# OnurBasci/TransformerBasedNavierStokeSolver

Measured on AMD Instinct MI355X. Metric: ns64_train_samples_per_s, higher is better.
Workload: dtype f32

## Files before the change

transformerbasednavierstokesolver_amd/csrc/pa2d_gemm.hip:

```cpp
#include "pa2d_gemm_common.h"
#include <string.h>


static Pa2dEnv read_env() {
    auto is = [](const char* n, const char* pre) { const char* e = getenv(n); return e && strncmp(e, pre, strlen(pre)) == 0; };
    auto num = [](const char* n, int dflt) { const char* e = getenv(n); return (e && e[0]) ? atoi(e) : dflt; };
    Pa2dEnv v;
    v.conv_halo = is("PA2D_CONV_HALO", "o") ? 0 : (is("PA2D_CONV_HALO", "f") ? 2 : 1);
    v.mc_big_off = is("PA2D_MC_BIG", "o") ? 1 : 0;
    v.kc_bk16 = num("PA2D_KC_BK", 0) == 16 ? 1 : 0;
    v.mc_bk = num("PA2D_MC_BK", 16) == 32 ? 32 : 16;
    v.mc_splits = num("PA2D_MC_SPLITS", 0);
    v.mcb_splits = num("PA2D_MCB_SPLITS", 0);
    v.lin_dw_split = is("PA2D_LIN_DW_SPLIT", "of") ? 0 : 1;
    v.lin_panel = is("PA2D_LIN_PANEL", "of") ? 0 : 1;
    v.lin_rowpanel = is("PA2D_LIN_ROWPANEL", "of") ? 0 : 1;
    v.lin_small_split = is("PA2D_LIN_SMALL_SPLIT", "of") ? 0 : 1;
    v.conv_mfma16 = num("PA2D_CONV_MFMA", 16) == 32 ? 0 : 1;
    v.split_big = num("PA2D_SPLIT_BIG", 1);
    v.slice_map = is("PA2D_SLICE_MAP", "l") ? 0 : 1;
    v.default_engine = is("PA2D_GEMM", "f") ? 0 : (is("PA2D_GEMM", "b") ? 2 : 1);
    return v;
}
static Pa2dEnv g_env = read_env();
const Pa2dEnv& pa2d_env() { return g_env; }
static int kc_bk(bool im2col, int Cin) {
    if (im2col && pa2d_env().kc_bk16) return 16;
    return (!im2col || (Cin % 32) == 0) ? 32 : 16;
}
KCTile kc_tile(int M, int N, bool im2col, int Cin) {
    const int tiles_m = ceil_div(M, 128);
    const long long t128 = (long long)tiles_m * ceil_div(N, 128);
    const long long t12864 = (long long)tiles_m * ceil_div(N, 64);
    const int bk = kc_bk(im2col, Cin);
    if (N > 64 && t128 >= 384) return {128, 128, bk};
    if (t12864 >= 384 || M <= 64) return {128, 64, bk};
    return {64, 64, bk};
}
bool use_split(int engine, int N, bool im2col, int Cin) {
    const int m = engine;
    if (m == 1) return im2col && N > 64 && (Cin % 32) == 0;
    if (m == 2) return N > 64 && (!im2col || (Cin % 32) == 0);
    return false;
}

int launch_kc(const KCParams& p_in, bool im2col, hipStream_t st, hipEvent_t ev0, hipEvent_t ev1) {
    KCParams p = p_in;
    if (!engine_ok(p.engine)) return PA2D_ERR_ARG;
    if (p.M <= 0 || p.N <= 0 || p.K <= 0) return PA2D_OK;
    if (!p.bias2) p.bias_split = 0x7fffffff;
    {
        const unsigned long long ab = ((unsigned long long)(p.M - 1) * p.lda + (im2col ? p.Cin : p.K)) * 4ull;
        const unsigned long long bb = ((unsigned long long)(p.N - 1) * p.ldb + p.K) * 4ull;
        if (ab >= 0xFFFFFFF0ull || bb >= 0xFFFFFFF0ull) return PA2D_ERR_UNSUPPORTED;
        p.a_bytes = (unsigned)ab;
        p.b_bytes = (unsigned)bb;
        const unsigned long long es = p.io_bf16 ? 2ull : 4ull;
        const unsigned long long cb = ((unsigned long long)(p.M - 1) * p.ldc + p.N) * es;
        const unsigned long long rb = p.res ? ((unsigned long long)(p.M - 1) * p.ldres + p.N) * es : 0ull;
        const unsigned long long xb = p.aux ? ((unsigned long long)(p.M - 1) * p.ldaux + p.N) * es : 0ull;
        if (cb >= 0xFFFFFFF0ull || rb >= 0xFFFFFFF0ull || xb >= 0xFFFFFFF0ull) return PA2D_ERR_UNSUPPORTED;
        p.c_bytes = (unsigned)cb; p.res_bytes = (unsigned)rb; p.aux_bytes = (unsigned)xb;
    }
    if ((p.K & 3) || (p.lda & 3) || (p.ldb & 3)) return PA2D_ERR_ARG;
    if (im2col && ((p.Cin & 15) || p.K != (p.taps == 27 ? 27 : 9) * p.Cin)) return PA2D_ERR_UNSUPPORTED;
    if (im2col && (p.epi != 0 || p.res)) return PA2D_ERR_ARG;
    if (ev0 && hipEventRecord(ev0, st) != hipSuccess) return PA2D_ERR_ARG;
    int rc;
    if (!im2col && p.wimg && rowpanel_applies(p)) {
        if (p.wsrc) {
            rc = launch_pack_weight_image(p.wsrc, p.wsn, p.wsk, p.wimg, p.N, p.K, st);
            if (rc) return rc;
        }
        KCParams pp = p;
        pp.M = p.M - p.M % 128;
        rc = launch_kc_rowpanel(pp, p.wimg, st);
        if (!rc && pp.M < p.M) {
            KCParams pt = p_in;
            pt.wimg = nullptr;
            pt.M = p.M - pp.M;
            pt.A = p.A + (size_t)pp.M * p.lda;
            pt.C = p.C + (size_t)pp.M * p.ldc;
            if (p.res) pt.res = p.res + (size_t)pp.M * p.ldres;
            if (p.aux) pt.aux = p.aux + (size_t)pp.M * p.ldaux;
            rc = launch_kc(pt, false, st);
        }
    } else if (panel_applies(p, im2col)) {
        KCParams pp = p;
        pp.M = p.M - p.M % 256;
        rc = launch_kc_panel(pp, st);
        if (!rc && pp.M < p.M) {
            KCParams pt = p_in;
            const size_t ea = p.io_bf16 ? 2 : 4, es = p.io_bf16 ? 2 : 4;
            pt.M = p.M - pp.M;
            pt.A = (const float*)((const char*)p.A + (size_t)pp.M * p.lda * ea);
            pt.C = (float*)((char*)p.C + (size_t)pp.M * p.ldc * es);
            if (p.res) pt.res = (const float*)((const char*)p.res + (size_t)pp.M * p.ldres * es);
            if (p.aux) pt.aux = (float*)((char*)p.aux + (size_t)pp.M * p.ldaux * es);
            rc = launch_kc(pt, false, st);
        }
    } else if (p.io_bf16 || use_split(p.engine, p.N, im2col, p.Cin)) rc = launch_kc_split(p, im2col, st);
    else if (kc_split_small_applies(p, im2col)) rc = launch_kc_split_small(p, st);
    else rc = launch_kc_f32(p, im2col, kc_tile(p.M, p.N, im2col, p.Cin), st);
    if (rc) return rc;
    if (ev1 && hipEventRecord(ev1, st) != hipSuccess) return PA2D_ERR_ARG;
    return PA2D_OK;
}

template <int TAPS>
__global__ void repack_kernel(const float* __restrict__ w0, const float* __restrict__ w1, float* __restrict__ dst,
                              int mode, int N, int K, int C, int Cin, int NK) {
    const long long idx = (long long)blockIdx.x * blockDim.x + threadIdx.x;
    if (mode == 0) {
        if (idx >= (long long)N * K) return;
        const int n = (int)(idx % N), k = (int)(idx / N);
        dst[idx] = w0[(size_t)n * K + k];
    } else if (mode == 1) {
        if (idx >= (long long)NK * C * TAPS * Cin) return;
        const int CH = K;
        const int c16 = (int)(idx % CH);
        const int tap = (int)((idx / CH) % TAPS);
        const int cic = (int)((idx / (TAPS * CH)) % (Cin / CH));
        const int co = (int)(idx / ((long long)Cin * TAPS));
        const int ci = cic * CH + c16;
        const float* src = co < C ? w0 : w1;
        dst[idx] = src[((size_t)(co % C) * Cin + ci) * TAPS + tap];
    } else {
        if (idx >= (long long)NK * C * TAPS * Cin) return;
        const int CH = K;
        const int c16 = (int)(idx % CH);
        const int tap = (int)((idx / CH) % TAPS);
        const int cic = (int)((idx / (TAPS * CH)) % (NK * C / CH));
        const int ci = (int)(idx / ((long long)NK * C * TAPS));
        const int co = cic * CH + c16;
        const float* src = co < C ? w0 : w1;
        dst[idx] = src[((size_t)(co % C) * Cin + ci) * TAPS + (TAPS - 1 - tap)];
    }
}

int launch_repack(const float* w0, const float* w1, float* dst, int mode, int N, int K, int C, int Cin, hipStream_t st,
                  int taps) {
    const int nk = w1 ? 2 : 1;
    const long long count = mode == 0 ? (long long)N * K : (long long)nk * C * taps * Cin;
    const dim3 grid((unsigned)ceil_div_ll(count, 256));
    if (taps == 27)
        hipLaunchKernelGGL(repack_kernel<27>, grid, dim3(256), 0, st, w0, w1, dst, mode, N, K, C, Cin, nk);
    else
        hipLaunchKernelGGL(repack_kernel<9>, grid, dim3(256), 0, st, w0, w1, dst, mode, N, K, C, Cin, nk);
    PA2D_CHECK_LAUNCH();
    return PA2D_OK;
}

static KCParams dense_fwd_params(const void* x, long long ldx, const float* w, long long ldw, const float* bias,
                                 const void* res, long long ldres, void* y, long long ldy, void* pre, long long ldpre, int M,
                                 int N, int K, int act, int engine, bool io_bf16) {
    KCParams p = {};
    p.engine = engine; p.io_bf16 = io_bf16 ? 1 : 0; p.apre = io_bf16 ? 1 : 0;
    p.aux_deriv = (act & PA2D_ACT_SAVE_DERIVATIVE_BIT) ? 1 : 0;
    act &= ~PA2D_ACT_SAVE_DERIVATIVE_BIT;
    p.A = (const float*)x; p.lda = ldx; p.B = w; p.ldb = ldw; p.C = (float*)y; p.ldc = ldy; p.bias = bias;
    p.res = (const float*)res; p.ldres = ldres; p.aux = (float*)pre; p.ldaux = ldpre; p.M = M; p.N = N; p.K = K; p.act = act;
    p.epi = (act != ACT_NONE ? EPI_ACT : 0) | (pre ? EPI_STORE_PRE : 0);
    return p;
}
static KCParams dense_bwd_data_params(const void* dy, long long lddy, const float* wt, const void* pre, long long ldpre,
                                      int act, void* dx, long long lddx, int M, int N, int K, int engine, bool io_bf16) {
    KCParams p = {};
    p.engine = engine; p.io_bf16 = io_bf16 ? 1 : 0; p.apre = io_bf16 ? 1 : 0;
    p.aux_deriv = (act & PA2D_ACT_SAVE_DERIVATIVE_BIT) ? 1 : 0;
    act &= ~PA2D_ACT_SAVE_DERIVATIVE_BIT;
    p.A = (const float*)dy; p.lda = lddy; p.B = wt; p.ldb = N; p.C = (float*)dx; p.ldc = lddx; p.M = M; p.N = K; p.K = N;
    p.aux = (float*)const_cast<void*>(pre); p.ldaux = ldpre; p.act = act;
    p.epi = (pre && act != ACT_NONE) ? EPI_MUL_DACT : 0;
// ... 126 lines not shown
```

transformerbasednavierstokesolver_amd/csrc/pa2d_internal.h:

```cpp
#pragma once
#include <hip/hip_runtime.h>
#include <stdint.h>

typedef float f32x16 __attribute__((ext_vector_type(16)));
typedef float f32x4 __attribute__((ext_vector_type(4)));

#define PA2D_OK 0
#define PA2D_ERR_ARG 1001
#define PA2D_ERR_UNSUPPORTED 1002
#define PA2D_ERR_WORKSPACE 1003

#define PA2D_CHECK_LAUNCH()                         \
    do {                                            \
        hipError_t e__ = hipGetLastError();         \
        if (e__ != hipSuccess) return (int)e__;     \
    } while (0)

enum { ACT_NONE = 0, ACT_GELU = 1, ACT_TANH = 2, ACT_SIGMOID = 3, ACT_RELU = 4, ACT_SOFTPLUS = 5,
       ACT_ELU = 6, ACT_SILU = 7 };

__device__ __forceinline__ float normal_cdf(float x, float& e_out) {
#pragma clang fp contract(off)
    const float z = fabsf(x) * 0.70710678118654752440f;
    const float t = __builtin_amdgcn_rcpf(fmaf(0.3275911f, z, 1.0f));
    float poly = fmaf(1.061405429f, t, -1.453152027f);
    poly = fmaf(poly, t, 1.421413741f);
    poly = fmaf(poly, t, -0.284496736f);
    poly = fmaf(poly, t, 0.254829592f);
    const float e = __builtin_amdgcn_exp2f(-z * z * 1.44269504088896340736f);
    e_out = e;
    const float hq = 0.5f * poly * t * e;
    return x < 0.f ? hq : 1.0f - hq;
}
__device__ __forceinline__ float gelu_exact(float x) {
#pragma clang fp contract(off)
    float e;
    return x * normal_cdf(x, e);
}
__device__ __forceinline__ float dgelu_exact(float x) {
#pragma clang fp contract(off)
    float e;
    const float cdf = normal_cdf(x, e);
    return fmaf(x * 0.39894228040143267794f, e, cdf);
}

__device__ __forceinline__ float act_fwd(int id, float x) {
    switch (id) {
        case ACT_GELU: return gelu_exact(x);
        case ACT_TANH: return tanhf(x);
        case ACT_SIGMOID: return 1.0f / (1.0f + expf(-x));
        case ACT_RELU: return x > 0.f ? x : 0.f;
        case ACT_SOFTPLUS: return x > 20.f ? x : log1pf(expf(x));
        case ACT_ELU: return x > 0.f ? x : expm1f(x);
        case ACT_SILU: return x / (1.0f + expf(-x));
        default: return x;
    }
}

__device__ __forceinline__ float act_bwd(int id, float x) {
    switch (id) {
        case ACT_GELU: return dgelu_exact(x);
        case ACT_TANH: { const float t = tanhf(x); return 1.0f - t * t; }
        case ACT_SIGMOID: { const float s = 1.0f / (1.0f + expf(-x)); return s * (1.0f - s); }
        case ACT_RELU: return x > 0.f ? 1.f : 0.f;
        case ACT_SOFTPLUS: return x > 20.f ? 1.f : 1.0f / (1.0f + expf(-x));
        case ACT_ELU: return x > 0.f ? 1.f : expf(x);
        case ACT_SILU: { const float s = 1.0f / (1.0f + expf(-x)); return s * (1.0f + x * (1.0f - s)); }
        default: return 1.f;
    }
}

__device__ __forceinline__ float wave_sum(float v) {
#pragma unroll
    for (int o = 32; o > 0; o >>= 1) v += __shfl_xor(v, o, 64);
    return v;
}
__device__ __forceinline__ float wave_max(float v) {
#pragma unroll
    for (int o = 32; o > 0; o >>= 1) v = fmaxf(v, __shfl_xor(v, o, 64));
    return v;
}

typedef unsigned int u32x4 __attribute__((ext_vector_type(4)));
#define OOB_OFF 0xFFFFFFFFu

__device__ __forceinline__ __amdgpu_buffer_rsrc_t make_rsrc(const float* base, unsigned bytes) {
    return __builtin_amdgcn_make_buffer_rsrc(const_cast<float*>(base), 0, bytes, 0x00020000);
}
__device__ __forceinline__ float4 buf_load4(__amdgpu_buffer_rsrc_t r, unsigned voff) {
    const u32x4 v = __builtin_amdgcn_raw_buffer_load_b128(r, voff, 0, 0);
    return make_float4(__uint_as_float(v.x), __uint_as_float(v.y), __uint_as_float(v.z), __uint_as_float(v.w));
}


__device__ __forceinline__ float buf_load1(__amdgpu_buffer_rsrc_t r, unsigned voff) {
    return __uint_as_float(__builtin_amdgcn_raw_buffer_load_b32(r, voff, 0, 0));
}
__device__ __forceinline__ void buf_store1(__amdgpu_buffer_rsrc_t r, unsigned voff, float v) {
    __builtin_amdgcn_raw_buffer_store_b32(__float_as_uint(v), r, voff, 0, 0);
}

__device__ __forceinline__ float2 buf_load2(__amdgpu_buffer_rsrc_t r, unsigned voff) {
    typedef unsigned int u32x2_ __attribute__((ext_vector_type(2)));
    const u32x2_ v = __builtin_amdgcn_raw_buffer_load_b64(r, voff, 0, 0);
    return make_float2(__uint_as_float(v.x), __uint_as_float(v.y));
}
__device__ __forceinline__ void buf_store4(__amdgpu_buffer_rsrc_t r, unsigned voff, float4 v) {
    u32x4 u = {__float_as_uint(v.x), __float_as_uint(v.y), __float_as_uint(v.z), __float_as_uint(v.w)};
    __builtin_amdgcn_raw_buffer_store_b128(u, r, voff, 0, 0);
}

#define PA2D_ACT_SAVE_DERIVATIVE_BIT 0x100

struct Pa2dEnv {
    int conv_halo;
    int mc_big_off;
    int kc_bk16;
    int mc_bk;
    int mc_splits;
    int mcb_splits;
    int lin_dw_split;
    int lin_panel;
    int conv_mfma16;
    int lin_small_split;
    int lin_rowpanel;
    int split_big;
    int slice_map;
    int default_engine;
};
const Pa2dEnv& pa2d_env();

static inline int pa2d_zero(void* p, size_t bytes, hipStream_t st) {
    if (!p || !bytes) return PA2D_OK;
    return (int)hipMemsetAsync(p, 0, bytes, st);
}
static inline int ceil_div(int a, int b) { return (a + b - 1) / b; }
static inline long long ceil_div_ll(long long a, long long b) { return (a + b - 1) / b; }

struct ReduceSegs { int nseg; long long begin[5]; float* dst[4]; };
int pa2d_launch_reduce_segs(const float* slab, int nslab, long long count, const ReduceSegs& segs, int accumulate,
                            hipStream_t st);

typedef __bf16 bf16_t;
template <typename T> struct Act;
template <> struct Act<float> {
    static constexpr unsigned ES = 4;
    static __device__ __forceinline__ float4 ld4(const float* p) { return *reinterpret_cast<const float4*>(p); }
    static __device__ __forceinline__ void st4(float* p, float4 v) { *reinterpret_cast<float4*>(p) = v; }
    static __device__ __forceinline__ float ld1(const float* p) { return *p; }
    static __device__ __forceinline__ float4 bld4(__amdgpu_buffer_rsrc_t r, unsigned off) { return buf_load4(r, off); }
    static __device__ __forceinline__ float2 bld2(__amdgpu_buffer_rsrc_t r, unsigned off) { return buf_load2(r, off); }
    static __device__ __forceinline__ float bld1(__amdgpu_buffer_rsrc_t r, unsigned off) { return buf_load1(r, off); }
    static __device__ __forceinline__ float bld1s(__amdgpu_buffer_rsrc_t r, unsigned off, unsigned soff) {
        return __uint_as_float(__builtin_amdgcn_raw_buffer_load_b32(r, off, soff, 0));
    }
    static __device__ __forceinline__ void bst4(__amdgpu_buffer_rsrc_t r, unsigned off, float4 v) { buf_store4(r, off, v); }
    static __device__ __forceinline__ void bst1(__amdgpu_buffer_rsrc_t r, unsigned off, float v) { buf_store1(r, off, v); }
};
__device__ __forceinline__ float bf16_bits_to_f32(unsigned short b) { return __uint_as_float((unsigned)b << 16); }
__device__ __forceinline__ unsigned short f32_to_bf16_bits(float x) {
    const bf16_t h = (bf16_t)x;
    return __builtin_bit_cast(unsigned short, h);
}
__device__ __forceinline__ unsigned pack_bf16x2(float lo, float hi) {
    return (unsigned)f32_to_bf16_bits(lo) | ((unsigned)f32_to_bf16_bits(hi) << 16);
}
template <> struct Act<bf16_t> {
    static constexpr unsigned ES = 2;
    static __device__ __forceinline__ float4 unpack4(uint2 q) {
        return make_float4(__uint_as_float(q.x << 16), __uint_as_float(q.x & 0xFFFF0000u), __uint_as_float(q.y << 16),
                           __uint_as_float(q.y & 0xFFFF0000u));
    }
    static __device__ __forceinline__ float4 ld4(const bf16_t* p) { return unpack4(*reinterpret_cast<const uint2*>(p)); }
    static __device__ __forceinline__ void st4(bf16_t* p, float4 v) {
        *reinterpret_cast<uint2*>(p) = make_uint2(pack_bf16x2(v.x, v.y), pack_bf16x2(v.z, v.w));
    }
    static __device__ __forceinline__ float ld1(const bf16_t* p) { return (float)*p; }
    static __device__ __forceinline__ float4 bld4(__amdgpu_buffer_rsrc_t r, unsigned off) {
        typedef unsigned int u32x2_ __attribute__((ext_vector_type(2)));
        const u32x2_ q = __builtin_amdgcn_raw_buffer_load_b64(r, off, 0, 0);
        return unpack4(make_uint2(q.x, q.y));
    }
    static __device__ __forceinline__ float2 bld2(__amdgpu_buffer_rsrc_t r, unsigned off) {
        const unsigned q = __builtin_amdgcn_raw_buffer_load_b32(r, off, 0, 0);
        return make_float2(__uint_as_float(q << 16), __uint_as_float(q & 0xFFFF0000u));
    }
    static __device__ __forceinline__ float bld1(__amdgpu_buffer_rsrc_t r, unsigned off) {
        return bf16_bits_to_f32(__builtin_amdgcn_raw_buffer_load_b16(r, off, 0, 0));
    }
    static __device__ __forceinline__ float bld1s(__amdgpu_buffer_rsrc_t r, unsigned off, unsigned soff) {
        return bf16_bits_to_f32(__builtin_amdgcn_raw_buffer_load_b16(r, off, soff, 0));
    }
    static __device__ __forceinline__ void bst4(__amdgpu_buffer_rsrc_t r, unsigned off, float4 v) {
        typedef unsigned int u32x2_ __attribute__((ext_vector_type(2)));
        const u32x2_ q = {pack_bf16x2(v.x, v.y), pack_bf16x2(v.z, v.w)};
        __builtin_amdgcn_raw_buffer_store_b64(q, r, off, 0, 0);
    }
    static __device__ __forceinline__ void bst1(__amdgpu_buffer_rsrc_t r, unsigned off, float v) {
        __builtin_amdgcn_raw_buffer_store_b16(f32_to_bf16_bits(v), r, off, 0, 0);
    }
};
__device__ __forceinline__ __amdgpu_buffer_rsrc_t make_rsrc_v(const void* base, unsigned bytes) {
    return __builtin_amdgcn_make_buffer_rsrc(const_cast<void*>(base), 0, bytes, 0x00020000);
}

__device__ __forceinline__ bool slice_decode(int xcd_map, int B, int heads, int nchunk, int& b, int& hh, int& chunk, int& bid) {
    const int total = B * heads * nchunk;
    int L;
    if (xcd_map) {
        const int per = (total + 7) >> 3;
        if ((int)(blockIdx.x >> 3) >= per) return false;
        L = (int)(blockIdx.x & 7) * per + (int)(blockIdx.x >> 3);
        if (L >= total) return false;
        hh = L % heads;
        chunk = (L / heads) % nchunk;
        b = L / (heads * nchunk);
    } else {
        L = (int)blockIdx.x;
        if (L >= total) return false;
        chunk = L % nchunk;
        hh = (L / nchunk) % heads;
        b = L / (nchunk * heads);
    }
    bid = (b * heads + hh) * nchunk + chunk;
    return true;
}
static inline int slice_grid(int total) { return ((total + 7) / 8) * 8; }
```

transformerbasednavierstokesolver_amd/csrc/pa2d_slice3.hip:

```cpp
#include "pa2d_slice_common.h"
#include "pa2d_bf16_split.h"
#include <stdlib.h>
#include <type_traits>

namespace {

__device__ __forceinline__ constexpr int kd(int s, int kq, int j) { return 32 * s + (j < 4 ? 4 * kq + j : 16 + 4 * kq + (j - 4)); }

template <typename T> struct RawK;
template <> struct RawK<float> { float4 a, b; };
template <> struct RawK<bf16_t> { u32x2 a, b; };
template <int D, typename T>
__device__ __forceinline__ void load_rawk(__amdgpu_buffer_rsrc_t r, unsigned off, int s, RawK<T>& x) {
    constexpr unsigned ES = Act<T>::ES;
    const int kq = (threadIdx.x >> 4) & 3;
    const bool ok0 = D == 16 || 32 * s + 4 * kq < D, ok1 = D == 16 || 32 * s + 16 + 4 * kq < D;
    const unsigned o0 = (off != OOB_OFF && ok0) ? off + 32 * s * ES : OOB_OFF;
    const unsigned o1 = (off != OOB_OFF && ok1) ? off + (D == 16 ? 4 : 32 * s + 16) * ES : OOB_OFF;
    if constexpr (sizeof(T) == 2) {
        x.a = __builtin_amdgcn_raw_buffer_load_b64(r, o0, 0, 0);
        x.b = __builtin_amdgcn_raw_buffer_load_b64(r, o1, 0, 0);
    } else {
        x.a = buf_load4(r, o0);
        x.b = buf_load4(r, o1);
    }
}
template <typename T>
__device__ __forceinline__ void rawk_planes(const RawK<T>& x, bf16x8 (&pl)[Planes<T>::ACT]) {
    if constexpr (sizeof(T) == 2) {
        const u32x4 q = {x.a.x, x.a.y, x.b.x, x.b.y};
        pl[0] = __builtin_bit_cast(bf16x8, q);
    } else {
        const f32x8 v = {x.a.x, x.a.y, x.a.z, x.a.w, x.b.x, x.b.y, x.b.z, x.b.w};
        split8<3>(v, pl);
    }
}

template <int D>
__device__ __forceinline__ void load_par8(const float* mat, int m, int M, int s, int kq, float scale, bf16x8 (&pl)[3]) {
    f32x8 x;
#pragma unroll
    for (int j = 0; j < 8; ++j) {
        const int d = kd(s, kq, j);
        x[j] = (m < M && d < D) ? mat[(size_t)m * D + d] * scale : 0.f;
    }
    split8<3>(x, pl);
}


template <int MT, typename T> struct W16 {
    static constexpr int NA = Planes<T>::ACT, NC = NA == 3 ? 3 : 2, MP = 16 * MT, PIMG = MP * 32;
    static constexpr int BIAS = 3 * PIMG, BYTES = BIAS + MP * 16;
    unsigned off[NC];
    const unsigned char* img;
    __device__ __forceinline__ void init(const unsigned char* base, int li, int kq) {
        img = base;
#pragma unroll
        for (int c = 0; c < NC; ++c) {
            const int pa = NA == 3 ? (c == 0 ? 0 : 1) : (c == 0 ? 0 : 2);
            const int pb = NA == 3 ? (c == 2 ? 2 : 0) : (c == 0 ? 1 : 2);
            off[c] = (unsigned)((kq < 2 ? pa : pb) * PIMG + li * 32 + (kq & 1) * 16);
        }
    }
    __device__ __forceinline__ f32x4 bias_n(int mt, int li) const {
        return *reinterpret_cast<const f32x4*>(img + BIAS + (16 * mt + li) * 16);
    }
    __device__ __forceinline__ f32x4 bias_t(int mt, int kq) const {
        return *reinterpret_cast<const f32x4*>(img + BIAS + (16 * mt + 4 * kq) * 4);
    }
    __device__ __forceinline__ bf16x8 frag(int c, int mt) const {
        return *reinterpret_cast<const bf16x8*>(img + off[c] + mt * 512);
    }
    static __device__ __forceinline__ void fill(unsigned char* base, const float* ws, const float* bs, int M, bool splat) {
        for (int i = threadIdx.x; i < MP; i += blockDim.x) {
            const float bv = i < M ? bs[i] : NEG_BIG;
            if (splat) *reinterpret_cast<f32x4*>(base + BIAS + i * 16) = (f32x4){bv, bv, bv, bv};
            else *reinterpret_cast<float*>(base + BIAS + i * 4) = bv;
        }
        for (int i = threadIdx.x; i < MP * 2; i += blockDim.x) {
            const int m = i >> 1, d0 = 8 * (i & 1);
            f32x8 v;
#pragma unroll
            for (int e = 0; e < 8; ++e) v[e] = m < M ? ws[(size_t)m * 16 + d0 + e] : 0.f;
            bf16x8 pl[3];
            split8<3>(v, pl);
#pragma unroll
            for (int q = 0; q < 3; ++q) *reinterpret_cast<bf16x8*>(base + q * PIMG + m * 32 + d0 * 2) = pl[q];
        }
        __syncthreads();
    }
    static __device__ __forceinline__ void combos(const bf16x8 (&xpl)[NA], int kq, bf16x8 (&xc)[NC]) {
        const bool lo = kq < 2;
        if constexpr (NA == 3) {
            const u32x4 x0 = __builtin_bit_cast(u32x4, xpl[0]), x1 = __builtin_bit_cast(u32x4, xpl[1]),
                        x2 = __builtin_bit_cast(u32x4, xpl[2]);
            u32x4 c0, c1, c2;
#pragma unroll
            for (int i = 0; i < 4; ++i) { c0[i] = lo ? x0[i] : x1[i]; c1[i] = lo ? x0[i] : x2[i]; c2[i] = lo ? x1[i] : x0[i]; }
            xc[0] = __builtin_bit_cast(bf16x8, c0); xc[1] = __builtin_bit_cast(bf16x8, c1); xc[2] = __builtin_bit_cast(bf16x8, c2);
        } else {
            const u32x4 x0 = __builtin_bit_cast(u32x4, xpl[0]);
            u32x4 c1;
#pragma unroll
            for (int i = 0; i < 4; ++i) c1[i] = lo ? x0[i] : 0u;
            xc[0] = xpl[0]; xc[1] = __builtin_bit_cast(bf16x8, c1);
        }
    }
};

template <int D> struct BCfg {
    static constexpr int KST = (D + 31) / 32;
    static constexpr int DT = (D + 15) / 16;
};

__device__ __forceinline__ bool slice3_decode(int B, int heads, int nchunk, int& b, int& hh, int& chunk, int& bid) {
    const int hpw = (int)(blockDim.x >> 6), ngroups = (heads + hpw - 1) / hpw;
    const int L = (int)blockIdx.x, hg = L % ngroups;
    chunk = (L / ngroups) % nchunk;
    b = L / (ngroups * nchunk);
    hh = hg * hpw + (int)(threadIdx.x >> 6);
    bid = (b * heads + hh) * nchunk + chunk;
    return hh < heads && b < B;
}

}

template <int D, int MT, typename T>
__global__ __launch_bounds__((MT <= 4 || D == 16) ? 512 : 256, (MT <= 4 || D == 16) ? 2 : 1) void scatter3_kernel(const SliceParams p) {
    constexpr int KST = BCfg<D>::KST, DT = BCfg<D>::DT;
    constexpr int NA = Planes<T>::ACT, NW = Planes<T>::WGT;
    constexpr unsigned ES = Act<T>::ES;
    constexpr bool K16 = D == 16;
    using W16T = W16<MT, T>;
    __shared__ __attribute__((aligned(16))) unsigned char wimg[K16 ? W16T::BYTES : 16];
    const int lane = threadIdx.x & 63, li = lane & 15, kq = lane >> 4;
    if constexpr (K16) W16T::fill(wimg, p.ws, p.bs, p.M, true);
    int b, hh, chunk, bid;
    if (!slice3_decode(p.B, p.heads, p.nchunk, b, hh, chunk, bid)) return;
    const float scale = LOG2E / (p.clamp ? clamp_tau(p.temperature[hh]) : p.temperature[hh]);
    const float esc = K16 ? scale : 1.0f;

    bf16x8 wsp[K16 ? 1 : MT][KST][3];
    W16T w16;
    if constexpr (K16) w16.init(wimg, li, kq);
    f32x4 bias[K16 ? 1 : MT];
    if constexpr (!K16) {
#pragma unroll
        for (int mt = 0; mt < MT; ++mt) {
            const int m = 16 * mt + li;
#pragma unroll
            for (int s = 0; s < KST; ++s) load_par8<D>(p.ws, m, p.M, s, kq, scale, wsp[mt][s]);
            const float bv = m < p.M ? p.bs[m] * scale : NEG_BIG;
            bias[mt] = (f32x4){bv, bv, bv, bv};
        }
    }
    f32x4 sacc[MT][DT];
    float nacc[MT];
#pragma unroll
    for (int mt = 0; mt < MT; ++mt) {
        nacc[mt] = 0.f;
#pragma unroll
        for (int dt = 0; dt < DT; ++dt) sacc[mt][dt] = (f32x4){0.f, 0.f, 0.f, 0.f};
    }
    const int p_begin = chunk * p.ppc;
    const int p_end = min(p.N, p_begin + p.ppc);
    const unsigned row0 = (unsigned)b * (unsigned)p.N + (unsigned)p_begin;
    const __amdgpu_buffer_rsrc_t rx = make_rsrc_v(p.xm, p.x_bytes);
    const __amdgpu_buffer_rsrc_t rv = make_rsrc_v(p.v, p.v_bytes);
    const unsigned ldxb = (unsigned)p.ldx * ES, ldvb = (unsigned)p.ldv * ES, hcol = (unsigned)(hh * D) * ES;
    const bool want_n = p.npart != nullptr;

    unsigned xo[2], vo = (row0 + 4 * kq) * ldvb + hcol + li * ES;
#pragma unroll
    for (int t = 0; t < 2; ++t) xo[t] = (row0 + 16 * t + li) * ldxb + hcol + (K16 ? 8 * (kq & 1) : 4 * kq) * ES;
    const unsigned xstep = 32u * ldxb, vstep = 32u * ldvb;
    unsigned vrow[8];
#pragma unroll
    for (int e = 0; e < 8; ++e) vrow[e] = (unsigned)(e < 4 ? e : 12 + e) * ldvb;

    RawK<T> xr[2][KST];
    float fv[DT][8];
    auto load_x = [&](auto tail, int n_left) {
#pragma unroll
        for (int t = 0; t < 2; ++t) {
            const unsigned off_ = (!decltype(tail)::value || 16 * t + li < n_left) ? xo[t] : OOB_OFF;
#pragma unroll
            for (int s = 0; s < KST; ++s) load_rawk<D, T>(rx, off_, s, xr[t][s]);
        }
    };
    auto load_v = [&](auto tail, int n_left) {
#pragma unroll
        for (int e = 0; e < 8; ++e) {
            const bool ok_ = !decltype(tail)::value || 4 * kq + (e < 4 ? e : 12 + e) < n_left;
#pragma unroll
            for (int dt = 0; dt < DT; ++dt) {
                const bool okd_ = 16 * dt + li < D;
                fv[dt][e] = Act<T>::bld1s(rv, (ok_ && okd_) ? vo + 16 * dt * ES : OOB_OFF, vrow[e]);
            }
        }
    };
    auto group = [&](auto tail, int n_left, int n_next) {
        constexpr bool TAIL = decltype(tail)::value;
        f32x4 w[2][MT];
#pragma unroll
        for (int t = 0; t < 2; ++t)
#pragma unroll
            for (int s = 0; s < KST; ++s) {
                bf16x8 xpl[NA];
                rawk_planes<T>(xr[t][s], xpl);
                if constexpr (K16) {
                    bf16x8 xc[W16T::NC];
                    W16T::combos(xpl, kq, xc);
#pragma unroll
                    for (int mt = 0; mt < MT; ++mt) {
                        f32x4 a = w16.bias_n(mt, li);
#pragma unroll
                        for (int c = W16T::NC - 1; c >= 0; --c) a = mfma_bf(xc[c], w16.frag(c, mt), a);
                        w[t][mt] = a;
                    }
                } else {
#pragma unroll
                    for (int mt = 0; mt < MT; ++mt) w[t][mt] = mfma_terms<NA, 3>(xpl, wsp[mt][s], s == 0 ? bias[mt] : w[t][mt]);
                }
            }
        xo[0] += xstep; xo[1] += xstep;
        if (n_next >= 32) load_x(std::false_type{}, n_next);
        else if (n_next > 0) load_x(std::true_type{}, n_next);
        f32x4 inv[2];
#pragma unroll
        for (int t = 0; t < 2; ++t) {
            float mx[4];
#pragma unroll
            for (int r = 0; r < 4; ++r) {
                mx[r] = w[t][0][r];
#pragma unroll
                for (int mt = 1; mt < MT; ++mt) mx[r] = fmaxf(mx[r], w[t][mt][r]);
            }
            row16_max4(mx[0], mx[1], mx[2], mx[3]);
            float sm[4];
#pragma unroll
            for (int r = 0; r < 4; ++r) {
                sm[r] = 0.f;
                const float nm = -mx[r] * esc;
#pragma unroll
                for (int mt = 0; mt < MT; ++mt) {
                    const float e = K16 ? ex2(fmaf(w[t][mt][r], esc, nm)) : ex2(w[t][mt][r] - mx[r]);
                    w[t][mt][r] = e;
                    sm[r] += e;
                }
            }
            row16_sum4(sm[0], sm[1], sm[2], sm[3]);
#pragma unroll
            for (int r = 0; r < 4; ++r) {
                const float iv = __builtin_amdgcn_rcpf(sm[r]);
                inv[t][r] = (!TAIL || 16 * t + 4 * kq + r < n_left) ? iv : 0.f;
            }
        }
        if (want_n) {
#pragma unroll
            for (int t = 0; t < 2; ++t)
#pragma unroll
                for (int mt = 0; mt < MT; ++mt)
#pragma unroll
                    for (int r = 0; r < 4; ++r) nacc[mt] = fmaf(w[t][mt][r], inv[t][r], nacc[mt]);
        }
        bf16x8 fp[DT][NA];
#pragma unroll
        for (int dt = 0; dt < DT; ++dt) {
            f32x8 f;
#pragma unroll
            for (int e = 0; e < 8; ++e) f[e] = NA == 1 ? fv[dt][e] : fv[dt][e] * inv[e >> 2][e & 3];
            split8<NA>(f, fp[dt]);
        }
        vo += vstep;
        if (n_next >= 32) load_v(std::false_type{}, n_next);
        else if (n_next > 0) load_v(std::true_type{}, n_next);
#pragma unroll
        for (int mt = 0; mt < MT; ++mt) {
            f32x8 wv;
#pragma unroll
            for (int e = 0; e < 8; ++e) wv[e] = NA == 1 ? w[e >> 2][mt][e & 3] * inv[e >> 2][e & 3] : w[e >> 2][mt][e & 3];
            bf16x8 wp[NW];
            split8<NW>(wv, wp);
#pragma unroll
            for (int dt = 0; dt < DT; ++dt) sacc[mt][dt] = mfma_terms<NW, NA>(wp, fp[dt], sacc[mt][dt]);
        }
    };

    int n_left = p_end - p_begin;
    if (n_left >= 32) { load_x(std::false_type{}, n_left); load_v(std::false_type{}, n_left); }
    else if (n_left > 0) { load_x(std::true_type{}, n_left); load_v(std::true_type{}, n_left); }
    for (; n_left >= 32; n_left -= 32) group(std::false_type{}, n_left, n_left - 32);
    if (n_left > 0) group(std::true_type{}, n_left, 0);

    float* so = p.spart + (size_t)bid * p.M * D;
#pragma unroll
    for (int mt = 0; mt < MT; ++mt)
#pragma unroll
        for (int dt = 0; dt < DT; ++dt)
#pragma unroll
            for (int r = 0; r < 4; ++r) {
                const int m = 16 * mt + 4 * kq + r, d = 16 * dt + li;
                if (m < p.M && d < D) so[m * D + d] = sacc[mt][dt][r];
            }
    if (want_n) {
#pragma unroll
        for (int mt = 0; mt < MT; ++mt) {
            const float v = kq_sum_swap(nacc[mt]);
            if (kq == 0 && 16 * mt + li < p.M) p.npart[(size_t)bid * p.M + 16 * mt + li] = v;
        }
    }
}

template <int D, int MT, typename T>
__global__ __launch_bounds__((MT <= 4 || D == 16) ? 512 : 256, (MT <= 4 || D == 16) ? 2 : 1) void deslice3_kernel(const DesliceParams p) {
    constexpr int KST = BCfg<D>::KST, DT = BCfg<D>::DT;
    constexpr int NA = Planes<T>::ACT, NW = Planes<T>::WGT;
    constexpr int MU = (MT + 1) / 2;
    constexpr unsigned ES = Act<T>::ES;
    constexpr bool K16 = D == 16;
    using W16T = W16<MT, T>;
    __shared__ __attribute__((aligned(16))) unsigned char wimg[K16 ? W16T::BYTES : 16];
    const int lane = threadIdx.x & 63, li = lane & 15, kq = lane >> 4;
    if constexpr (K16) W16T::fill(wimg, p.ws, p.bs, p.M, false);
    int b, hh, chunk, bid;
    if (!slice3_decode(p.B, p.heads, p.nchunk, b, hh, chunk, bid)) return;
    const float scale = LOG2E / (p.clamp ? clamp_tau(p.temperature[hh]) : p.temperature[hh]);
    const float esc = K16 ? scale : 1.0f;

    bf16x8 wsp[K16 ? 1 : MT][KST][3];
    W16T w16;
    if constexpr (K16) w16.init(wimg, li, kq);
    f32x4 bias[K16 ? 1 : MT];
    bf16x8 op[MU][DT][3];
    const float* ob = p.o + (size_t)(b * p.heads + hh) * p.M * D;
    if constexpr (!K16) {
#pragma unroll
        for (int mt = 0; mt < MT; ++mt) {
#pragma unroll
            for (int s = 0; s < KST; ++s) load_par8<D>(p.ws, 16 * mt + li, p.M, s, kq, scale, wsp[mt][s]);
#pragma unroll
            for (int r = 0; r < 4; ++r) {
                const int mr = 16 * mt + 4 * kq + r;
                bias[mt][r] = mr < p.M ? p.bs[mr] * scale : NEG_BIG;
            }
        }
    }
#pragma unroll
    for (int u = 0; u < MU; ++u)
#pragma unroll
        for (int dt = 0; dt < DT; ++dt) {
            f32x8 x;
            const int d = 16 * dt + li;
#pragma unroll
            for (int e = 0; e < 8; ++e) {
                const int m = e < 4 ? 32 * u + 4 * kq + e : 32 * u + 12 + 4 * kq + e;
                x[e] = (m < p.M && d < D) ? ob[(size_t)m * D + d] : 0.f;
            }
            split8<3>(x, op[u][dt]);
        }
    const int p_begin = chunk * p.ppc;
    const int p_end = min(p.N, p_begin + p.ppc);
    const unsigned row0 = (unsigned)b * (unsigned)p.N + (unsigned)p_begin;
    const __amdgpu_buffer_rsrc_t rx = make_rsrc_v(p.xm, p.x_bytes);
    const __amdgpu_buffer_rsrc_t ry = make_rsrc_v(p.y, p.y_bytes);
    const unsigned ldxb = (unsigned)p.ldx * ES, ldyb = (unsigned)p.ldy * ES, hcol = (unsigned)(hh * D) * ES;
    unsigned xo[2], yo[2];
#pragma unroll
    for (int t = 0; t < 2; ++t) {
        xo[t] = (row0 + 16 * t + li) * ldxb + hcol + (K16 ? 8 * (kq & 1) : 4 * kq) * ES;
        yo[t] = (row0 + 16 * t + li) * ldyb + hcol + 4 * kq * ES;
    }
    const unsigned xstep = 32u * ldxb, ystep = 32u * ldyb;

    RawK<T> xr[2][KST];
    auto load_x = [&](auto tail, int n_left) {
#pragma unroll
        for (int t = 0; t < 2; ++t) {
            const unsigned off_ = (!decltype(tail)::value || 16 * t + li < n_left) ? xo[t] : OOB_OFF;
#pragma unroll
            for (int s = 0; s < KST; ++s) load_rawk<D, T>(rx, off_, s, xr[t][s]);
        }
    };
    auto group = [&](auto tail, int n_left, int n_next) {
        constexpr bool TAIL = decltype(tail)::value;
        f32x4 w[2][MT];
#pragma unroll
        for (int t = 0; t < 2; ++t)
#pragma unroll
            for (int s = 0; s < KST; ++s) {
                bf16x8 xpl[NA];
                rawk_planes<T>(xr[t][s], xpl);
                if constexpr (K16) {
                    bf16x8 xc[W16T::NC];
                    W16T::combos(xpl, kq, xc);
#pragma unroll
                    for (int mt = 0; mt < MT; ++mt) {
                        f32x4 a = w16.bias_t(mt, kq);
#pragma unroll
                        for (int c = W16T::NC - 1; c >= 0; --c) a = mfma_bf(w16.frag(c, mt), xc[c], a);
                        w[t][mt] = a;
                    }
                } else {
#pragma unroll
                    for (int mt = 0; mt < MT; ++mt) w[t][mt] = mfma_terms<3, NA>(wsp[mt][s], xpl, s == 0 ? bias[mt] : w[t][mt]);
                }
            }
        xo[0] += xstep; xo[1] += xstep;
        if (n_next >= 32) load_x(std::false_type{}, n_next);
        else if (n_next > 0) load_x(std::true_type{}, n_next);
#pragma unroll
        for (int t = 0; t < 2; ++t) {
            float mx = w[t][0][0];
#pragma unroll
            for (int mt = 0; mt < MT; ++mt)
#pragma unroll
                for (int r = 0; r < 4; ++r) mx = fmaxf(mx, w[t][mt][r]);
            mx = kq_max_swap(mx);
            float sm = 0.f;
            const float nm = -mx * esc;
#pragma unroll
            for (int mt = 0; mt < MT; ++mt)
#pragma unroll
                for (int r = 0; r < 4; ++r) {
                    const float e = K16 ? ex2(fmaf(w[t][mt][r], esc, nm)) : ex2(w[t][mt][r] - mx);
                    w[t][mt][r] = e;
                    sm += e;
                }
            sm = kq_sum_swap(sm);
            const float inv = __builtin_amdgcn_rcpf(sm);
            f32x4 yacc[DT];
#pragma unroll
            for (int dt = 0; dt < DT; ++dt) yacc[dt] = (f32x4){0.f, 0.f, 0.f, 0.f};
#pragma unroll
            for (int u = 0; u < MU; ++u) {
                f32x8 wv;
#pragma unroll
                for (int e = 0; e < 4; ++e) {
                    wv[e] = w[t][2 * u][e];
                    wv[4 + e] = (2 * u + 1 < MT) ? w[t][(2 * u + 1 < MT) ? 2 * u + 1 : 0][e] : 0.f;
                }
                bf16x8 wp[NW];
                split8<NW>(wv, wp);
#pragma unroll
                for (int dt = 0; dt < DT; ++dt) yacc[dt] = mfma_terms<3, NW>(op[u][dt], wp, yacc[dt]);
            }
            const bool pv = !TAIL || 16 * t + li < n_left;
#pragma unroll
            for (int dt = 0; dt < DT; ++dt) {
                const bool okd = 16 * dt + 4 * kq < D;
                Act<T>::bst4(ry, (pv && okd) ? yo[t] + 16 * dt * ES : OOB_OFF,
                             make_float4(yacc[dt][0] * inv, yacc[dt][1] * inv, yacc[dt][2] * inv, yacc[dt][3] * inv));
            }
        }
        yo[0] += ystep; yo[1] += ystep;
#pragma unroll
        for (int i = 0; i < 96; ++i) { __builtin_amdgcn_sched_group_barrier(0x008, 1, 0); __builtin_amdgcn_sched_group_barrier(0x002, 4, 0); }
    };
    int n_left = p_end - p_begin;
    if (n_left >= 32) load_x(std::false_type{}, n_left);
    else if (n_left > 0) load_x(std::true_type{}, n_left);
    for (; n_left >= 32; n_left -= 32) group(std::false_type{}, n_left, n_left - 32);
    if (n_left > 0) group(std::true_type{}, n_left, 0);
}

static int slice3_hpw(int B, int heads, int nchunk, int mt, int D) {
    int hpw = (mt <= 4 || D == 16) ? 8 : 4;
    if (hpw > heads) hpw = heads;
    while (hpw > 1 && (long long)B * nchunk * ((heads + hpw - 1) / hpw) < 256) hpw >>= 1;
    return hpw;
}
template <int D, int MT>
static int launch_scatter3_t(const SliceParams& p, dim3 grid, dim3 block, bool bf, hipStream_t st) {
    if (bf) hipLaunchKernelGGL((scatter3_kernel<D, MT, bf16_t>), grid, block, 0, st, p);
    else hipLaunchKernelGGL((scatter3_kernel<D, MT, float>), grid, block, 0, st, p);
    return PA2D_OK;
}
template <int D, int MT>
static int launch_deslice3_t(const DesliceParams& p, dim3 grid, dim3 block, bool bf, hipStream_t st) {
    if (bf) hipLaunchKernelGGL((deslice3_kernel<D, MT, bf16_t>), grid, block, 0, st, p);
    else hipLaunchKernelGGL((deslice3_kernel<D, MT, float>), grid, block, 0, st, p);
    return PA2D_OK;
}

int launch_scatter3(const SliceParams& p, int D, int mt, bool bf, hipStream_t st) {
    const int hpw = slice3_hpw(p.B, p.heads, p.nchunk, mt, D);
    const dim3 grid(p.B * p.nchunk * ((p.heads + hpw - 1) / hpw)), block(64 * hpw);
#define CALL_S3(D_, MT_) launch_scatter3_t<D_, MT_>(p, grid, block, bf, st)
    SLICE_DISPATCH_D(CALL_S3)
    return PA2D_ERR_UNSUPPORTED;
}

int launch_deslice3(const DesliceParams& p, int D, int mt, bool bf, hipStream_t st) {
    const int hpw = slice3_hpw(p.B, p.heads, p.nchunk, mt, D);
    const dim3 grid(p.B * p.nchunk * ((p.heads + hpw - 1) / hpw)), block(64 * hpw);
#define CALL_D3(D_, MT_) launch_deslice3_t<D_, MT_>(p, grid, block, bf, st)
    SLICE_DISPATCH_D(CALL_D3)
    return PA2D_ERR_UNSUPPORTED;
}
```

Before: 70.84.

## Stage slice scatter/deslice inputs through per-wave LDS ring via async buffer loads

Adds an LDS ring buffer per wave, filled by buffer_load...lds DMA instructions, that prefetches x and v rows two groups ahead in the fp32 D=32 scatter kernel and x rows in the deslice kernel. The goal is to hide global-load latency and free the registers that held prefetched raw rows. By default the scatter kernel uses the ring and the deslice ring stays behind an env switch. It adds dynamic shared memory use, which can reduce occupancy, and relies on inline asm with manual m0 and waitcnt handling.

Result: no change. 71.04, median of 5 (+0.3%).

```diff
diff --git a/transformerbasednavierstokesolver_amd/csrc/pa2d_gemm.hip b/transformerbasednavierstokesolver_amd/csrc/pa2d_gemm.hip
--- a/transformerbasednavierstokesolver_amd/csrc/pa2d_gemm.hip
+++ b/transformerbasednavierstokesolver_amd/csrc/pa2d_gemm.hip
@@ -19,6 +19,7 @@
     v.conv_mfma16 = num("PA2D_CONV_MFMA", 16) == 32 ? 0 : 1;
     v.split_big = num("PA2D_SPLIT_BIG", 1);
     v.slice_map = is("PA2D_SLICE_MAP", "l") ? 0 : 1;
+    v.slice_stage = is("PA2D_SLICE_STAGE", "r") ? 0 : (is("PA2D_SLICE_STAGE", "l") ? 1 : 2);
     v.default_engine = is("PA2D_GEMM", "f") ? 0 : (is("PA2D_GEMM", "b") ? 2 : 1);
     return v;
 }
diff --git a/transformerbasednavierstokesolver_amd/csrc/pa2d_internal.h b/transformerbasednavierstokesolver_amd/csrc/pa2d_internal.h
--- a/transformerbasednavierstokesolver_amd/csrc/pa2d_internal.h
+++ b/transformerbasednavierstokesolver_amd/csrc/pa2d_internal.h
@@ -126,6 +126,7 @@
     int lin_rowpanel;
     int split_big;
     int slice_map;
+    int slice_stage;
     int default_engine;
 };
 const Pa2dEnv& pa2d_env();
diff --git a/transformerbasednavierstokesolver_amd/csrc/pa2d_slice3.hip b/transformerbasednavierstokesolver_amd/csrc/pa2d_slice3.hip
--- a/transformerbasednavierstokesolver_amd/csrc/pa2d_slice3.hip
+++ b/transformerbasednavierstokesolver_amd/csrc/pa2d_slice3.hip
@@ -36,6 +36,56 @@
     }
 }
 
+constexpr unsigned RING_TENSOR = 32 * 128;
+
+__device__ __forceinline__ constexpr unsigned ring_swz(unsigned r) {
+    const unsigned h = r >> 1;
+    return (h & 1u) | ((h & 2u) << 1) | ((h & 4u) >> 1);
+}
+__device__ __forceinline__ constexpr unsigned ring_at(unsigned r, unsigned q) { return r * 128u + ((q ^ ring_swz(r)) << 4); }
+__device__ __forceinline__ unsigned ring_src(unsigned lane, unsigned i, unsigned ldb) {
+    const unsigned r = 8u * i + (lane >> 3);
+    return (lane >> 3) * ldb + (((lane & 7u) ^ ring_swz(r)) << 4);
+}
+__device__ __forceinline__ u32x4 ring_desc(const void* base, unsigned bytes) {
+    const unsigned long long a = (unsigned long long)base;
+    return (u32x4){(unsigned)a, (unsigned)(a >> 32) & 0xFFFFu, bytes, 0x00020000u};
+}
+__device__ __forceinline__ void ring_dma4(u32x4 rs, unsigned v0, unsigned v1, unsigned soff, unsigned rstep, unsigned dst) {
+    unsigned keep;
+    const unsigned s1 = soff + rstep, s2 = s1 + rstep, s3 = s2 + rstep;
+    asm volatile("s_waitcnt lgkmcnt(0)\n\t"
+                 "s_nop 4\n\t"
+                 "s_mov_b32 %0, m0\n\t"
+                 "s_mov_b32 m0, %8\n\t"
+                 "s_nop 0\n\t"
+                 "buffer_load_dwordx4 %1, %3, %4 offen lds\n\t"
+                 "s_add_u32 m0, m0, 0x400\n\t"
+                 "s_nop 0\n\t"
+                 "buffer_load_dwordx4 %2, %3, %5 offen lds\n\t"
+                 "s_add_u32 m0, m0, 0x400\n\t"
+                 "s_nop 0\n\t"
+                 "buffer_load_dwordx4 %1, %3, %6 offen lds\n\t"
+                 "s_add_u32 m0, m0, 0x400\n\t"
+                 "s_nop 0\n\t"
+                 "buffer_load_dwordx4 %2, %3, %7 offen lds\n\t"
+                 "s_mov_b32 m0, %0"
+                 : "=&s"(keep)
+                 : "v"(v0), "v"(v1), "s"(rs), "s"(soff), "s"(s1), "s"(s2), "s"(s3), "s"(dst)
+                 : "memory", "scc");
+}
+template <int N> __device__ __forceinline__ void ring_wait() { asm volatile("s_waitcnt vmcnt(%0)" ::"n"(N) : "memory"); }
+template <typename T, int KST>
+__device__ __forceinline__ void ring_read_x(const unsigned char* slot, unsigned xa, unsigned xb, RawK<T> (&xr)[2][KST]) {
+    if constexpr (sizeof(T) == 4) {
+#pragma unroll
+        for (int t = 0; t < 2; ++t) {
+            xr[t][0].a = *reinterpret_cast<const float4*>(slot + xa + t * 2048);
+            xr[t][0].b = *reinterpret_cast<const float4*>(slot + xb + t * 2048);
+        }
+    }
+}
+
 template <int D>
 __device__ __forceinline__ void load_par8(const float* mat, int m, int M, int s, int kq, float scale, bf16x8 (&pl)[3]) {
     f32x8 x;
@@ -125,8 +175,10 @@
 
 }
 
-template <int D, int MT, typename T>
-__global__ __launch_bounds__((MT <= 4 || D == 16) ? 512 : 256, (MT <= 4 || D == 16) ? 2 : 1) void scatter3_kernel(const SliceParams p) {
+template <int D, int MT, typename T, bool ST>
+__device__ __forceinline__ void scatter3_body(const SliceParams& p) {
+    static_assert(!ST || (D == 32 && sizeof(T) == 4), "the LDS ring is built for fp32 rows of 32 channels");
+    extern __shared__ __attribute__((aligned(16))) unsigned char ring[];
     constexpr int KST = BCfg<D>::KST, DT = BCfg<D>::DT;
     constexpr int NA = Planes<T>::ACT, NW = Planes<T>::WGT;
     constexpr unsigned ES = Act<T>::ES;
@@ -178,6 +230,20 @@
 #pragma unroll
     for (int e = 0; e < 8; ++e) vrow[e] = (unsigned)(e < 4 ? e : 12 + e) * ldvb;
 
+    constexpr unsigned RSLOT = 2 * RING_TENSOR;
+    const unsigned rbase = ST ? (unsigned)__builtin_amdgcn_readfirstlane((int)(threadIdx.x >> 6)) * (2 * RSLOT) : 0u;
+    const unsigned rlds = (unsigned)(size_t)ring + rbase;
+    const u32x4 dxd = ring_desc(p.xm, p.x_bytes), dvd = ring_desc(p.v, p.v_bytes);
+    const unsigned sx0 = ring_src(lane, 0, ldxb) + hcol, sx1 = ring_src(lane, 1, ldxb) + hcol;
+    const unsigned sv0 = ring_src(lane, 0, ldvb) + hcol, sv1 = ring_src(lane, 1, ldvb) + hcol;
+    const unsigned xa = ring_at(li, kq), xb = ring_at(li, 4 + kq);
+    unsigned va[DT][2];
+#pragma unroll
+    for (int dt = 0; dt < DT; ++dt)
+#pragma unroll
+        for (int cb = 0; cb < 2; ++cb) va[dt][cb] = ring_at(4 * kq + 2 * cb, 4 * dt + (li >> 2)) - 2 * cb * 128 + (li & 3) * 4;
+    unsigned rslot = 0, dsx = row0 * ldxb, dsv = row0 * ldvb;
+
     RawK<T> xr[2][KST];
     float fv[DT][8];
     auto load_x = [&](auto tail, int n_left) {
@@ -199,8 +265,14 @@
             }
         }
     };
-    auto group = [&](auto tail, int n_left, int n_next) {
+    auto group = [&](auto tail, auto stage, int n_left, int n_next) {
         constexpr bool TAIL = decltype(tail)::value;
+        constexpr int STG = decltype(stage)::value;
+        const unsigned char* slot = ring + rbase + rslot * RSLOT;
+        if constexpr (STG != 0) {
+            ring_wait<STG == 1 ? 8 : 0>();
+            ring_read_x(slot, xa, xb, xr);
+        }
         f32x4 w[2][MT];
 #pragma unroll
         for (int t = 0; t < 2; ++t)
@@ -224,8 +296,13 @@
                 }
             }
         xo[0] += xstep; xo[1] += xstep;
-        if (n_next >= 32) load_x(std::false_type{}, n_next);
-        else if (n_next > 0) load_x(std::true_type{}, n_next);
+        if constexpr (STG == 1) {
+            if (n_left >= 96) ring_dma4(dxd, sx0, sx1, dsx, 8u * ldxb, rlds + rslot * RSLOT);
+            dsx += xstep;
+        } else {
+            if (n_next >= 32) load_x(std::false_type{}, n_next);
+            else if (n_next > 0) load_x(std::true_type{}, n_next);
+        }
         f32x4 inv[2];
 #pragma unroll
         for (int t = 0; t < 2; ++t) {
@@ -264,6 +341,15 @@
 #pragma unroll
                     for (int r = 0; r < 4; ++r) nacc[mt] = fmaf(w[t][mt][r], inv[t][r], nacc[mt]);
         }
+        if constexpr (STG != 0) {
+#pragma unroll
+            for (int e = 0; e < 8; ++e) {
+                const int c = e < 4 ? e : 12 + e;
+#pragma unroll
+                for (int dt = 0; dt < DT; ++dt)
+                    fv[dt][e] = *reinterpret_cast<const float*>(slot + RING_TENSOR + va[dt][(c >> 1) & 1] + c * 128);
+            }
+        }
         bf16x8 fp[DT][NA];
 #pragma unroll
         for (int dt = 0; dt < DT; ++dt) {
@@ -273,8 +359,14 @@
             split8<NA>(f, fp[dt]);
         }
         vo += vstep;
-        if (n_next >= 32) load_v(std::false_type{}, n_next);
-        else if (n_next > 0) load_v(std::true_type{}, n_next);
+        if constexpr (STG == 1) {
+            if (n_left >= 96) ring_dma4(dvd, sv0, sv1, dsv, 8u * ldvb, rlds + rslot * RSLOT + RING_TENSOR);
+            dsv += vstep;
+            rslot ^= 1u;
+        } else {
+            if (n_next >= 32) load_v(std::false_type{}, n_next);
+            else if (n_next > 0) load_v(std::true_type{}, n_next);
+        }
 #pragma unroll
         for (int mt = 0; mt < MT; ++mt) {
             f32x8 wv;
@@ -287,11 +379,30 @@
         }
     };
 
+    using Stg0 = std::integral_constant<int, 0>;
     int n_left = p_end - p_begin;
-    if (n_left >= 32) { load_x(std::false_type{}, n_left); load_v(std::false_type{}, n_left); }
-    else if (n_left > 0) { load_x(std::true_type{}, n_left); load_v(std::true_type{}, n_left); }
-    for (; n_left >= 32; n_left -= 32) group(std::false_type{}, n_left, n_left - 32);
-    if (n_left > 0) group(std::true_type{}, n_left, 0);
+    if constexpr (ST) {
+        if (n_left >= 32) {
+            ring_dma4(dxd, sx0, sx1, dsx, 8u * ldxb, rlds);
+            ring_dma4(dvd, sv0, sv1, dsv, 8u * ldvb, rlds + RING_TENSOR);
+            if (n_left >= 64) {
+                ring_dma4(dxd, sx0, sx1, dsx + xstep, 8u * ldxb, rlds + RSLOT);
+                ring_dma4(dvd, sv0, sv1, dsv + vstep, 8u * ldvb, rlds + RSLOT + RING_TENSOR);
+            }
+            dsx += 2 * xstep; dsv += 2 * vstep;
+            for (; n_left >= 64; n_left -= 32) group(std::false_type{}, std::integral_constant<int, 1>{}, n_left, n_left - 32);
+            group(std::false_type{}, std::integral_constant<int, 2>{}, n_left, n_left - 32);
+            n_left -= 32;
+        } else if (n_left > 0) {
+            load_x(std::true_type{}, n_left); load_v(std::true_type{}, n_left);
+            __builtin_amdgcn_s_waitcnt(0x0F70);
+        }
+    } else {
+        if (n_left >= 32) { load_x(std::false_type{}, n_left); load_v(std::false_type{}, n_left); }
+        else if (n_left > 0) { load_x(std::true_type{}, n_left); load_v(std::true_type{}, n_left); }
+        for (; n_left >= 32; n_left -= 32) group(std::false_type{}, Stg0{}, n_left, n_left - 32);
+    }
+    if (n_left > 0) group(std::true_type{}, Stg0{}, n_left, 0);
 
     float* so = p.spart + (size_t)bid * p.M * D;
 #pragma unroll
@@ -313,7 +424,18 @@
 }
 
 template <int D, int MT, typename T>
-__global__ __launch_bounds__((MT <= 4 || D == 16) ? 512 : 256, (MT <= 4 || D == 16) ? 2 : 1) void deslice3_kernel(const DesliceParams p) {
+__global__ __launch_bounds__((MT <= 4 || D == 16) ? 512 : 256, (MT <= 4 || D == 16) ? 2 : 1) void scatter3_kernel(const SliceParams p) {
+    scatter3_body<D, MT, T, false>(p);
+}
+template <int D, int MT>
+__global__ __launch_bounds__((MT <= 4 || D == 16) ? 512 : 256, (MT <= 4 || D == 16) ? 2 : 1) void scatter3_ring_kernel(const SliceParams p) {
+    scatter3_body<D, MT, float, true>(p);
+}
+
+template <int D, int MT, typename T, bool ST>
+__device__ __forceinline__ void deslice3_body(const DesliceParams& p) {
+    static_assert(!ST || (D == 32 && sizeof(T) == 4), "the LDS ring is built for fp32 rows of 32 channels");
+    extern __shared__ __attribute__((aligned(16))) unsigned char ring[];
     constexpr int KST = BCfg<D>::KST, DT = BCfg<D>::DT;
     constexpr int NA = Planes<T>::ACT, NW = Planes<T>::WGT;
     constexpr int MU = (MT + 1) / 2;
@@ -372,6 +494,12 @@
         yo[t] = (row0 + 16 * t + li) * ldyb + hcol + 4 * kq * ES;
     }
     const unsigned xstep = 32u * ldxb, ystep = 32u * ldyb;
+    const unsigned rbase = ST ? (unsigned)__builtin_amdgcn_readfirstlane((int)(threadIdx.x >> 6)) * (3 * RING_TENSOR) : 0u;
+    const unsigned rlds = (unsigned)(size_t)ring + rbase;
+    const u32x4 dxd = ring_desc(p.xm, p.x_bytes);
+    const unsigned sx0 = ring_src(lane, 0, ldxb) + hcol, sx1 = ring_src(lane, 1, ldxb) + hcol;
+    const unsigned xa = ring_at(li, kq), xb = ring_at(li, 4 + kq);
+    unsigned rslot = 0, wslot = 2, dsx = row0 * ldxb;
 
     RawK<T> xr[2][KST];
     auto load_x = [&](auto tail, int n_left) {
@@ -382,8 +510,25 @@
             for (int s = 0; s < KST; ++s) load_rawk<D, T>(rx, off_, s, xr[t][s]);
         }
     };
-    auto group = [&](auto tail, int n_left, int n_next) {
+    auto group = [&](auto tail, auto stage, int n_left, int n_next) {
         constexpr bool TAIL = decltype(tail)::value;
+        constexpr int STG = decltype(stage)::value;
+        if constexpr (STG == 1) {
+            if (n_left >= 96) {
+                ring_dma4(dxd, sx0, sx1, dsx, 8u * ldxb, rlds + wslot * RING_TENSOR);
+                ring_wait<8>();
+            } else {
+                ring_wait<4>();
+            }
+            dsx += xstep;
+            wslot = wslot == 2 ? 0 : wslot + 1;
+        } else if constexpr (STG == 2) {
+            ring_wait<0>();
+        }
+        if constexpr (STG != 0) {
+            ring_read_x(ring + rbase + rslot * RING_TENSOR, xa, xb, xr);
+            rslot = rslot == 2 ? 0 : rslot + 1;
+        }
         f32x4 w[2][MT];
 #pragma unroll
         for (int t = 0; t < 2; ++t)
@@ -407,8 +552,10 @@
                 }
             }
         xo[0] += xstep; xo[1] += xstep;
-        if (n_next >= 32) load_x(std::false_type{}, n_next);
-        else if (n_next > 0) load_x(std::true_type{}, n_next);
+        if constexpr (STG != 1) {
+            if (n_next >= 32) load_x(std::false_type{}, n_next);
+            else if (n_next > 0) load_x(std::true_type{}, n_next);
+        }
 #pragma unroll
         for (int t = 0; t < 2; ++t) {
             float mx = w[t][0][0];
@@ -457,11 +604,35 @@
 #pragma unroll
         for (int i = 0; i < 96; ++i) { __builtin_amdgcn_sched_group_barrier(0x008, 1, 0); __builtin_amdgcn_sched_group_barrier(0x002, 4, 0); }
     };
+    using Stg0 = std::integral_constant<int, 0>;
     int n_left = p_end - p_begin;
-    if (n_left >= 32) load_x(std::false_type{}, n_left);
-    else if (n_left > 0) load_x(std::true_type{}, n_left);
-    for (; n_left >= 32; n_left -= 32) group(std::false_type{}, n_left, n_left - 32);
-    if (n_left > 0) group(std::true_type{}, n_left, 0);
+    if constexpr (ST) {
+        if (n_left >= 32) {
+            ring_dma4(dxd, sx0, sx1, dsx, 8u * ldxb, rlds);
+            if (n_left >= 64) ring_dma4(dxd, sx0, sx1, dsx + xstep, 8u * ldxb, rlds + RING_TENSOR);
+            dsx += 2 * xstep;
+            for (; n_left >= 64; n_left -= 32) group(std::false_type{}, std::integral_constant<int, 1>{}, n_left, n_left - 32);
+            group(std::false_type{}, std::integral_constant<int, 2>{}, n_left, n_left - 32);
+            n_left -= 32;
+        } else if (n_left > 0) {
+            load_x(std::true_type{}, n_left);
+            __builtin_amdgcn_s_waitcnt(0x0F70);
+        }
+    } else {
+        if (n_left >= 32) load_x(std::false_type{}, n_left);
+        else if (n_left > 0) load_x(std::true_type{}, n_left);
+        for (; n_left >= 32; n_left -= 32) group(std::false_type{}, Stg0{}, n_left, n_left - 32);
+    }
+    if (n_left > 0) group(std::true_type{}, Stg0{}, n_left, 0);
+}
+
+template <int D, int MT, typename T>
+__global__ __launch_bounds__((MT <= 4 || D == 16) ? 512 : 256, (MT <= 4 || D == 16) ? 2 : 1) void deslice3_kernel(const DesliceParams p) {
+    deslice3_body<D, MT, T, false>(p);
+}
+template <int D, int MT>
+__global__ __launch_bounds__((MT <= 4 || D == 16) ? 512 : 256, (MT <= 4 || D == 16) ? 2 : 1) void deslice3_ring_kernel(const DesliceParams p) {
+    deslice3_body<D, MT, float, true>(p);
 }
 
 static int slice3_hpw(int B, int heads, int nchunk, int mt, int D) {
@@ -470,14 +641,35 @@
     while (hpw > 1 && (long long)B * nchunk * ((heads + hpw - 1) / hpw) < 256) hpw >>= 1;
     return hpw;
 }
+template <int D, int MT> constexpr bool ring_built() { return D == 32 && MT <= 4; }
 template <int D, int MT>
 static int launch_scatter3_t(const SliceParams& p, dim3 grid, dim3 block, bool bf, hipStream_t st) {
+    if constexpr (ring_built<D, MT>()) {
+        if (!bf && pa2d_env().slice_stage != 0) {
+            const int smem = (int)(block.x >> 6) * 4 * (int)RING_TENSOR;
+            const hipError_t e = hipFuncSetAttribute(reinterpret_cast<const void*>(&scatter3_ring_kernel<D, MT>),
+                                                     hipFuncAttributeMaxDynamicSharedMemorySize, smem);
+            if (e != hipSuccess) return (int)e;
+            hipLaunchKernelGGL((scatter3_ring_kernel<D, MT>), grid, block, smem, st, p);
+            return PA2D_OK;
+        }
+    }
     if (bf) hipLaunchKernelGGL((scatter3_kernel<D, MT, bf16_t>), grid, block, 0, st, p);
     else hipLaunchKernelGGL((scatter3_kernel<D, MT, float>), grid, block, 0, st, p);
     return PA2D_OK;
 }
 template <int D, int MT>
 static int launch_deslice3_t(const DesliceParams& p, dim3 grid, dim3 block, bool bf, hipStream_t st) {
+    if constexpr (ring_built<D, MT>()) {
+        if (!bf && pa2d_env().slice_stage == 1) {
+            const int smem = (int)(block.x >> 6) * 3 * (int)RING_TENSOR;
+            const hipError_t e = hipFuncSetAttribute(reinterpret_cast<const void*>(&deslice3_ring_kernel<D, MT>),
+                                                     hipFuncAttributeMaxDynamicSharedMemorySize, smem);
+            if (e != hipSuccess) return (int)e;
+            hipLaunchKernelGGL((deslice3_ring_kernel<D, MT>), grid, block, smem, st, p);
+            return PA2D_OK;
+        }
+    }
     if (bf) hipLaunchKernelGGL((deslice3_kernel<D, MT, bf16_t>), grid, block, 0, st, p);
     else hipLaunchKernelGGL((deslice3_kernel<D, MT, float>), grid, block, 0, st, p);
     return PA2D_OK;
```
